# danieleschmidt/DiffFE-Physics-Lab

Measured on NVIDIA B200. Metric: fem_fwd_adjoint_solves_per_s, higher is better.
Workload: dtype f64

## Files before the change

difffe_physics_lab_b200/csrc/dfe_1d_pipe.cu:

```cuda
#include <cstdint>
#include <cstdlib>

#include "dfe_internal.h"

namespace {

#include "dfe_1d_common.cuh"

constexpr unsigned long long SENT = 0xFFFFFFFFFFFFFFFFull;
constexpr int NLMAX = 4;
constexpr int MISC_BYTES = 4096;

struct PP {
  int nn, G, chg, NG, slotd;
  long long B;
  const double* hs;
  const double* rh;
  const double* X;
  const double* in0;
  long long ld0;
  const double* in1;
  long long ld1;
  double* out;
  long long ldo;
// ... 64 lines not shown
        const long long t0 = clock64();
        while (clock64() - t0 < backoff) {}
      }
    }
  }
  s = __longlong_as_double(static_cast<long long>(a));
  m = __longlong_as_double(static_cast<long long>(b));
}

constexpr long long WAIT_LIMIT = 4000000000ll;
__device__ __forceinline__ bool mbar_try(uint64_t* bar, uint32_t parity) {
  uint32_t ok;
  asm volatile(
      "{\n\t.reg .pred p;\n\t"
      "mbarrier.try_wait.parity.shared::cta.b64 p, [%1], %2;\n\t"
      "selp.u32 %0, 1, 0, p;\n\t}"
      : "=r"(ok)
      : "r"(smem_u32(bar)), "r"(parity)
      : "memory");
  return ok != 0;
}
__device__ __forceinline__ bool mbar_test(uint64_t* bar, uint32_t parity) {
  uint32_t ok;
  asm volatile(
      "{\n\t.reg .pred p;\n\t"
      "mbarrier.test_wait.parity.shared::cta.b64 p, [%1], %2;\n\t"
      "selp.u32 %0, 1, 0, p;\n\t}"
      : "=r"(ok)
      : "r"(smem_u32(bar)), "r"(parity)
      : "memory");
  return ok != 0;
}
__device__ __noinline__ void mbar_wait_slow(uint64_t* bar, uint32_t parity, int* err, int* dead) {
  const long long t0 = clock64();
  int spins = 0;
  while (!mbar_try(bar, parity)) {
    if ((++spins & 63) == 0) {
      if (*reinterpret_cast<volatile int*>(dead)) return;
      if (clock64() - t0 > WAIT_LIMIT) {
        *reinterpret_cast<volatile int*>(dead) = 1;
        *reinterpret_cast<volatile int*>(err) = 1;
        return;
      }
    }
  }
}
__device__ __forceinline__ void mbar_wait_b(uint64_t* bar, uint32_t parity, int* err, int* dead) {
  if (!mbar_test(bar, parity)) mbar_wait_slow(bar, parity, err, dead);
}
__device__ __forceinline__ void mbar_arrive(uint64_t* bar) {
  asm volatile("mbarrier.arrive.shared::cta.b64 _, [%0];" ::"r"(smem_u32(bar)) : "memory");
}

template <bool BWD, int R, bool FULL, bool MF>
__device__ __forceinline__ void phase_a(double* buf, const double* ub, const double (&hs)[R + 1], int nin, int nst,
                                        bool ownsL, double sc, double& S, double& Wc, double& Lq) {
#pragma unroll
  for (int j = 0; j < R; ++j) {
    double in;
    if (MF) {
      const double diff = (FULL || j < nst) ? ub[j] - buf[j] : 0.0;
      Lq = fma(diff, diff, Lq);
      in = (FULL || j < nin) ? sc * diff : 0.0;
      if (!FULL && j == 0 && ownsL) in = 0.0;
      if (FULL || j < nst) buf[j] = in;
    } else {
      in = (FULL || j < nin) ? buf[j] : 0.0;
    }
    double F = BWD ? in : fma(in, hs[j + 1], in * hs[j]);
    if (!FULL && j == 0 && ownsL) F = 0.0;
    if (!BWD && (FULL || j < nst)) buf[j] = Wc;
    S += F;
    Wc = fma(hs[j + 1], S, Wc);
  }
}

template <bool BWD, int R, bool FULL, bool SK, bool KEEP>
__device__ __forceinline__ void phase_b(double* buf, const double* ub, const double (&hs)[R + 1], const double (&rh)[R + 1],
                                        double X0, int nin, int nst, bool ownsL, double c0, double kaph, double a0,
                                        double b0, double& S1, double& W1, double& D) {
  double S = 0.0, Wc = 0.0;
  double kp = SK ? 0.0 : kdiv(kaph, hs[0], rh[0]);
  double t = fma(b0, X0, a0);
#pragma unroll
  for (int j = 0; j < R; ++j) {
    double g = 0.0, Wt;
    if (BWD) {
      g = (FULL || j < nin) ? buf[j] : 0.0;
      if (!FULL && j == 0 && ownsL) g = 0.0;
      Wt = Wc;
      S += g;
      Wc = fma(hs[j + 1], S, Wc);
    } else {
      Wt = (FULL || j < nst) ? buf[j] : 0.0;
    }
    const double x0 = fma(-c0, Wt, t);
    t = fma(b0, hs[j + 1], t);
    double v1;
    if (SK) {
      v1 = __dmul_rn(rh[j + 1], x0);
    } else {
      const double ki = kdiv(kaph, hs[j + 1], rh[j + 1]);
      v1 = __dmul_rn(two_sum_err(kp, ki), x0);
      kp = ki;
    }
    if (BWD) {
      const double uj = (FULL || j < nst) ? ub[j] : 0.0;
      D = fma(g + v1, uj, D);
    }
    if (KEEP && (FULL || j < nst)) buf[j] = fma(-c0, W1, x0);
    S1 += v1;
    W1 = fma(hs[j + 1], S1, W1);
  }
}

template <bool BWD, int R, bool FULL>
__device__ __forceinline__ void phase_c(double* buf, const double (&hs)[R + 1], double X0, int nst, double a1, double b1) {
  double t = fma(b1, X0, a1);
#pragma unroll
  for (int j = 0; j < R; ++j) {
    if (FULL || j < nst) {
      const double xv = buf[j] + t;
      buf[j] = BWD ? fma(xv, hs[j], xv * hs[j + 1]) : xv;
    }
    t = fma(b1, hs[j + 1], t);
  }
}

template <int W, int NR>
struct Ctl {
  uint64_t full[NR];
  uint64_t outr[NR];
  uint64_t ufull[4];
  uint64_t ufree[4];
  uint64_t tot[2][2];
  uint64_t cf[2][2];
  double cfa[2][2][2];
  double red[2][W];
  double redL[2][W];
  double sc[2][4];
  int dead;
};

template <bool BWD, int W, int NR, int LB, int LC, bool MF>
__device__ __forceinline__ void fold_warp(const PP& p, Ctl<W, NR>* ctl, double2* pt, int lane, int c, int grp, int nIt,
                                          int nTot, const int ST) {
  constexpr int WP = W | 1;
  const int LAG = ST == 0 ? LB : LB + LC;
  const int G = p.G, GP = G + 2;
  const bool LR = p.bcL && p.bcR;
  const double rXtot = 1.0 / p.Xtot;
  const bool lift = (!BWD && ST == 0);
  const double ga = (lift && LR) ? (p.gR - p.gL) * rXtot : 0.0;
  const double gb = lift ? (p.bcL ? p.gL : p.gR) : 0.0;
  const long long sstep = p.NG;
  long long sF = grp + static_cast<long long>(1 - LAG) * sstep;
  long long sP = grp + static_cast<long long>(ST == 0 ? 0 : -LB) * sstep;
  const bool ends = BWD && c == 0;
  double ccur = 0.0, khcur = 0.0, uLcur = 0.0, uRcur = 0.0;
  {
    const int f = 1 - LAG;
    if (f >= 0 && f < nIt) {
      const double* ck = p.ck + (p.per_sample ? 2 * sF : 0);
      ccur = ck[0];
      khcur = ck[1];
      if (ends) { uLcur = p.in1[sF * p.ld1]; uRcur = p.in1[sF * p.ld1 + p.nn - 1]; }
    }
  }
  if (lane == 0) mbar_arrive(&ctl->cf[ST][0]);

  for (int it = 0; it < nTot; ++it) {
    const int par = it & 1, nxt = par ^ 1;
    const uint32_t ph = (it >> 1) & 1;
    const int f = it + 1 - LAG;
    const bool vf = f >= 0 && f < nIt;
    const unsigned long long* base = p.part + ((sF * 2 + ST) * G) * 2;
    unsigned long long ra[3], rb[3];
#pragma unroll
    for (int l = 0; l < 3; ++l) {
      const int ci = lane + 32 * l;
      ra[l] = rb[l] = SENT;
      if (vf && ci < G) ld_pair(base + 2 * ci, ra[l], rb[l]);
    }
    double cnx = 0.0, khnx = 0.0, uLnx = 0.0, uRnx = 0.0;
    if (f + 1 >= 0 && f + 1 < nIt) {
      const long long sN = sF + sstep;
      const double* ck = p.ck + (p.per_sample ? 2 * sN : 0);
      cnx = ck[0];
      khnx = ck[1];
      if (ends) { uLnx = p.in1[sN * p.ld1]; uRnx = p.in1[sN * p.ld1 + p.nn - 1]; }
    }
    mbar_wait_b(&ctl->tot[ST][par], ph, p.err, &ctl->dead);
    {
      double2* P = pt + static_cast<size_t>(ST * 2 + par) * (32 * WP) + lane * WP;
      double es[W], em[W];
      double rs = 0.0, rm = 0.0;
#pragma unroll
      for (int k = 0; k < W; ++k) {
// ... 28 lines not shown
        for (int d = 16; d > 0; d >>= 1) a += __shfl_xor_sync(0xffffffffu, a, d);
        if (jp >= 0 && jp < nIt && lane == 0) p.gkpart[sP * GP + c] = a;
      }
    }
    if (vf) {
      double Sx = 0.0, Mx = 0.0, St = 0.0, Mt = 0.0;
#pragma unroll
      for (int l = 0; l < 3; ++l) {
        const int ci = lane + 32 * l;
        if (ci < G) {
          double sv, mv;
          poll_pair(base + 2 * ci, ra[l], rb[l], sv, mv, p.err, &ctl->dead, p.backoff);
          St += sv; Mt += mv;
          if (ci < c) { Sx += sv; Mx += mv; }
        }
      }
      for (int l0 = 96; l0 < G; l0 += 32) {
        const int ci = lane + l0;
        if (ci < G) {
          double sv, mv;
          poll_pair(base + 2 * ci, SENT, SENT, sv, mv, p.err, &ctl->dead, p.backoff);
          St += sv; Mt += mv;
          if (ci < c) { Sx += sv; Mx += mv; }
        }
      }
#pragma unroll
      for (int d = 16; d > 0; d >>= 1) {
        Sx += __shfl_xor_sync(0xffffffffu, Sx, d);
        Mx += __shfl_xor_sync(0xffffffffu, Mx, d);
        St += __shfl_xor_sync(0xffffffffu, St, d);
        Mt += __shfl_xor_sync(0xffffffffu, Mt, d);
      }
      const double cc = ccur;
      const double Wtot = fma(St, p.Xtot, Mt);
      const double C = LR ? Wtot * rXtot : (p.bcL ? St : 0.0);
      const double A = gb + (p.bcL ? 0.0 : cc * Wtot) - cc * Mx;
      const double Bc = ga + cc * (C - Sx);
      if (lane == 0) {
        ctl->cfa[ST][nxt][0] = A;
        ctl->cfa[ST][nxt][1] = Bc;
        ctl->sc[nxt][2 * ST] = cc;
        if (ST == 0) ctl->sc[nxt][1] = khcur;
        if (ends) p.gkpart[sF * GP + G + ST] = C * (uRcur - uLcur) - St * uRcur;
      }
    }
    ccur = cnx; khcur = khnx; uLcur = uLnx; uRcur = uRnx;
    sF += sstep;
    sP += sstep;
    __syncwarp();
    if (lane == 0) mbar_arrive(&ctl->cf[ST][nxt]);
  }
}

template <bool BWD, int R, int W, int LB, int LC, bool SK, bool MF, bool OUT, int PF>
__global__ void __launch_bounds__(32 * (W + 3), (W >= 8 ? 1 : 2)) k1d_pipe(const PP p) {
  constexpr int LCO = OUT ? LC : 0;
  constexpr int NR = LB + LCO + 2 + PF;
  constexpr int NRU = MF ? LB + 2 : 2;
  static_assert(W <= 16 && LB >= 1 && LC >= 1 && NRU <= 4 && (!MF || BWD) && (OUT || BWD), "layout");
  static_assert(sizeof(Ctl<W, NR>) <= MISC_BYTES, "misc region");
  extern __shared__ __align__(16) unsigned char smem_raw[];
  Ctl<W, NR>* ctl = reinterpret_cast<Ctl<W, NR>*>(smem_raw);
  constexpr int WP = W | 1;
  double* ring = reinterpret_cast<double*>(smem_raw + MISC_BYTES);
  double* uring = ring + static_cast<size_t>(NR) * p.slotd;
  double2* pt = reinterpret_cast<double2*>(uring + static_cast<size_t>(BWD ? NRU : 0) * p.slotd);

  const int tid = threadIdx.x, lane = tid & 31, warp = tid >> 5;
  const int G = p.G, nn = p.nn;
  const int c = blockIdx.x % G, grp = blockIdx.x / G;
  const int n0 = c * p.chg;
  const int len = min(nn, n0 + p.chg) - n0;
  const int nIt = static_cast<int>((p.B - grp + p.NG - 1) / p.NG);
  const int nTot = nIt + LB + LC;
  const bool have_out = OUT && (p.out != nullptr);
  const int slotd = p.slotd;
  const int mis0c = static_cast<int>(((reinterpret_cast<uintptr_t>(p.in0) >> 3) + n0) & 1);
  const int mis1c = BWD ? static_cast<int>(((reinterpret_cast<uintptr_t>(p.in1) >> 3) + n0) & 1) : 0;
  const int ld0p = static_cast<int>(p.ld0 & 1), ld1p = static_cast<int>(p.ld1 & 1), ngp = p.NG & 1, grpp = grp & 1;
  auto mis0_of = [&](int j) { return mis0c ^ (ld0p & (grpp ^ (j & ngp))); };
  auto mis1_of = [&](int j) { return mis1c ^ (ld1p & (grpp ^ (j & ngp))); };

  if (tid == 0) {
    for (int k = 0; k < NR; ++k) { mbar_init_raw(&ctl->full[k], 1); mbar_init_raw(&ctl->outr[k], W); }
    for (int k = 0; k < 4; ++k) {
      mbar_init_raw(&ctl->ufull[k], 1);
      mbar_init_raw(&ctl->ufree[k], W);
    }
    for (int k = 0; k < 2; ++k)
      for (int s = 0; s < 2; ++s) { mbar_init_raw(&ctl->tot[s][k], W); mbar_init_raw(&ctl->cf[s][k], 1); }
    fence_mbar_init();
    ctl->dead = 0;
  }
  __syncthreads();

  if (warp < W) {
    const int tb = tid * R;
    const int nin = max(0, min(R, min(len, nn - (p.bcR ? 1 : 0) - n0) - tb));
    const int nst = max(0, min(R, len - tb));
    const bool ownsL = p.bcL && c == 0 && tid == 0;
    const bool ownsR = p.bcR && c == G - 1 && tb <= len - 1 && len - 1 < tb + R;
    const bool full = __all_sync(0xffffffffu, (nin == R) && (nst == R) && !ownsL && !ownsR);
    double hs[R + 1], rh[R + 1];
#pragma unroll
    for (int j = 0; j <= R; ++j) {
      const int e = n0 - 1 + tb + j;
      const bool ex = (e >= 0 && e < nn - 1 && tb + j <= len);
      hs[j] = ex ? p.hs[e] : 0.0;
      rh[j] = ex ? p.rh[e] : 0.0;
    }
    if (SK) {
      const double kaph = 0.5 * p.kappa[0];
      double kp = kdiv(kaph, hs[0], rh[0]);
#pragma unroll
      for (int j = 0; j < R; ++j) {
        const double ki = kdiv(kaph, hs[j + 1], rh[j + 1]);
        rh[j + 1] = two_sum_err(kp, ki);
        kp = ki;
      }
    }
    const double X0 = p.X[min(n0 + tb, nn - 1)];
    const double Xe = p.X[min(n0 + min(tb + R, len), nn - 1)];
    double q0s[LB - 1], q0m[LB - 1], q1s[LC - 1], q1m[LC - 1];
#pragma unroll
    for (int k = 0; k < LB - 1; ++k) q0s[k] = q0m[k] = 0.0;
#pragma unroll
    for (int k = 0; k < LC - 1; ++k) q1s[k] = q1m[k] = 0.0;
    const int pidx = (tid / W) * WP + tid % W;
    double2* pt0 = pt + pidx;
    double2* pt1 = pt + 2 * 32 * WP + pidx;

    int slotA = 0, roundA = 0;
    for (int it = 0; it < nTot; ++it) {
      const int par = it & 1;
      const uint32_t ph = (it >> 1) & 1;
      {
        double S = 0.0, Wc = 0.0, Lq = 0.0;
        if (it < nIt) {
          double* buf = ring + slotA * slotd + mis0_of(it) + tb;
          mbar_wait_b(&ctl->full[slotA], roundA, p.err, &ctl->dead);
          const double* ub = nullptr;
          if (MF) {
            const int us = it % NRU;
            ub = uring + us * slotd + mis1_of(it) + tb;
            mbar_wait_b(&ctl->ufull[us], (it / NRU) & 1, p.err, &ctl->dead);
          }
          if (full) phase_a<BWD, R, true, MF>(buf, ub, hs, nin, nst, ownsL, p.mf_scale, S, Wc, Lq);
          else phase_a<BWD, R, false, MF>(buf, ub, hs, nin, nst, ownsL, p.mf_scale, S, Wc, Lq);
        }
        pt0[par * 32 * WP] = make_double2(S, fma(-S, Xe, Wc));
        if (MF) {
#pragma unroll
          for (int d = 16; d > 0; d >>= 1) Lq += __shfl_xor_sync(0xffffffffu, Lq, d);
          if (lane == 0) ctl->redL[par][warp] = Lq;
        }
        __syncwarp();
        if (lane == 0) mbar_arrive(&ctl->tot[0][par]);
      }
      {
        const int jB = it - LB;
        int slotB = slotA - LB;
        if (slotB < 0) slotB += NR;
        double S1 = 0.0, W1 = 0.0, D = 0.0;
        mbar_wait_b(&ctl->cf[0][par], ph, p.err, &ctl->dead);
        const bool act = jB >= 0 && jB < nIt;
        if (act) {
          double* buf = ring + slotB * slotd + mis0_of(jB) + tb;
          const double c0 = ctl->sc[par][0], kaph = ctl->sc[par][1];
          const double a0 = fma(-c0, q0m[LB - 2], ctl->cfa[0][par][0]);
          const double b0 = fma(-c0, q0s[LB - 2], ctl->cfa[0][par][1]);
          const double* ub = nullptr;
          if (BWD) {
            const int us = jB % NRU;
            ub = uring + us * slotd + mis1_of(jB) + tb;
            mbar_wait_b(&ctl->ufull[us], (jB / NRU) & 1, p.err, &ctl->dead);
          }
          if (full) phase_b<BWD, R, true, SK, OUT>(buf, ub, hs, rh, X0, nin, nst, ownsL, c0, kaph, a0, b0, S1, W1, D);
          else phase_b<BWD, R, false, SK, OUT>(buf, ub, hs, rh, X0, nin, nst, ownsL, c0, kaph, a0, b0, S1, W1, D);
          if (!OUT && MF) fence_async_smem();
        }
        {
          const double2 e0 = pt0[(par ^ 1) * 32 * WP];
#pragma unroll
          for (int k = LB - 2; k > 0; --k) { q0s[k] = q0s[k - 1]; q0m[k] = q0m[k - 1]; }
          q0s[0] = e0.x;
          q0m[0] = e0.y;
        }
        pt1[par * 32 * WP] = make_double2(S1, fma(-S1, Xe, W1));
        if (BWD) {
#pragma unroll
          for (int d = 16; d > 0; d >>= 1) D += __shfl_xor_sync(0xffffffffu, D, d);
          if (lane == 0) ctl->red[par][warp] = D;
        }
        __syncwarp();
        if (lane == 0) {
          mbar_arrive(&ctl->tot[1][par]);
          if (BWD && act) mbar_arrive(&ctl->ufree[jB % NRU]);
          if (!OUT && act) mbar_arrive(&ctl->outr[slotB]);
        }
      }
      {
        const int jC = it - LB - LC;
        mbar_wait_b(&ctl->cf[1][par], ph, p.err, &ctl->dead);
        if (OUT && jC >= 0 && jC < nIt) {
          int slotC = slotA - LB - LC;
          if (slotC < 0) slotC += NR;
          if (have_out) {
            double* buf = ring + slotC * slotd + mis0_of(jC) + tb;
            const double c1 = ctl->sc[par][2];
            const double a1 = fma(-c1, q1m[LC - 2], ctl->cfa[1][par][0]);
            const double b1 = fma(-c1, q1s[LC - 2], ctl->cfa[1][par][1]);
            if (full) {
              phase_c<BWD, R, true>(buf, hs, X0, nst, a1, b1);
            } else {
              phase_c<BWD, R, false>(buf, hs, X0, nst, a1, b1);
              if (ownsL) buf[0] = BWD ? 0.0 : p.gL;
              if (ownsR) buf[len - 1 - tb] = BWD ? 0.0 : p.gR;
            }
            fence_async_smem();
          }
          __syncwarp();
          if (lane == 0) mbar_arrive(&ctl->outr[slotC]);
        }
        {
          const double2 e1 = pt1[(par ^ 1) * 32 * WP];
#pragma unroll
          for (int k = LC - 2; k > 0; --k) { q1s[k] = q1s[k - 1]; q1m[k] = q1m[k - 1]; }
          q1s[0] = e1.x;
          q1m[0] = e1.y;
        }
      }
      if (++slotA == NR) { slotA = 0; roundA ^= 1; }
    }
  } else if (warp <= W + 1) {
    fold_warp<BWD, W, NR, LB, LC, MF>(p, ctl, pt, lane, c, grp, nIt, nTot, warp - W);
  } else {
    const long long last_s = p.B - 1;
    auto load_row = [&](const double* rowbase, long long ld, long long s, double* dst, uint64_t* mb) {
      const double* g = rowbase + s * ld + n0;
      const int mis = static_cast<int>((reinterpret_cast<uintptr_t>(g) >> 3) & 1);
      int cnt = (mis + len + 1) & ~1;
      const bool clip = (s == last_s && c == G - 1 && ((mis + len) & 1));
      if (clip) cnt -= 2;
      if (lane == 0) {
        if (clip) dst[mis + len - 1] = g[len - 1];
        mbar_arrive_expect_tx(mb, 8u * static_cast<uint32_t>(cnt));
        if (cnt) bulk_g2s(dst, g - mis, 8u * cnt, mb);
      }
    };
    for (int j = 0; j < NR && j < nIt; ++j)
      load_row(p.in0, p.ld0, grp + static_cast<long long>(j) * p.NG, ring + j * slotd, &ctl->full[j]);
    if (BWD)
      for (int j = 0; j < NRU && j < nIt; ++j)
        load_row(p.in1, p.ld1, grp + static_cast<long long>(j) * p.NG, uring + j * slotd, &ctl->ufull[j]);

    int slotC = 0, roundC = 0;
    for (int it = LB; it < nTot; ++it) {
      if (BWD) {
        const int jb = it - LB;
        if (jb < nIt) {
          const int us = jb % NRU;
          mbar_wait_b(&ctl->ufree[us], (jb / NRU) & 1, p.err, &ctl->dead);
          if (jb + NRU < nIt)
            load_row(p.in1, p.ld1, grp + static_cast<long long>(jb + NRU) * p.NG, uring + us * slotd, &ctl->ufull[us]);
        }
      }
      const int jc = it - LB - LCO;
      if (jc >= 0 && jc < nIt) {
        mbar_wait_b(&ctl->outr[slotC], roundC, p.err, &ctl->dead);
        if (have_out) {
          const long long s = grp + static_cast<long long>(jc) * p.NG;
          double* go = p.out + s * p.ldo + n0;
          const double* ssrc = ring + slotC * slotd;
          const Seg qo = make_seg(go, len);
          if (lane == 0) {
            if (qo.body) bulk_s2g(go + qo.head, ssrc + qo.mis + qo.head, 8u * qo.body);
            bulk_commit();
          } else if (lane == 1) {
            if (qo.head) go[0] = ssrc[qo.mis];
          } else if (lane == 2) {
            if (qo.tail) go[len - 1] = ssrc[qo.mis + len - 1];
          }
          if (lane == 0) bulk_wait_read0();
          __syncwarp();
        }
        if (jc + NR < nIt)
          load_row(p.in0, p.ld0, grp + static_cast<long long>(jc + NR) * p.NG, ring + slotC * slotd, &ctl->full[slotC]);
        if (++slotC == NR) { slotC = 0; roundC ^= 1; }
      }
    }
    if (lane == 0) bulk_wait_all0();
  }
}

__global__ void k1d_pipe_ck(const double* kappa, long long n, double* ck, unsigned* ticket) {
  const long long s = blockIdx.x * static_cast<long long>(blockDim.x) + threadIdx.x;
  if (s == 0) *ticket = 0u;
  if (s < n) {
    const double k = kappa[s];
    ck[2 * s] = 2.0 / k;
    ck[2 * s + 1] = 0.5 * k;
  }
}

constexpr int GK_SPB = 1024;
__global__ void __launch_bounds__(256) k1d_pipe_gk(const double* part, const double* lpart, const double* kappa,
                                                   long long B, int GP, int G, int per_sample, double lsc, double* out,
                                                   double* loss_out, double* blk, unsigned* ticket) {
  if (per_sample) {
    const long long s = blockIdx.x * static_cast<long long>(blockDim.x) + threadIdx.x;
    if (s < B) {
      double a = 0.0;
      for (int g = 0; g < GP; ++g) a += part[s * GP + g];
      out[s] = -a / kappa[s];
      if (lpart) {
        double q = 0.0;
        for (int c = 0; c < G; ++c) q += lpart[s * G + c];
        loss_out[s] = lsc * q;
      }
    }
    return;
  }
  __shared__ double sh[2][256];
  __shared__ int is_last;
  const int tid = threadIdx.x;
  double a = 0.0, l = 0.0;
  for (int k = 0; k < GK_SPB / 256; ++k) {
    const long long s = static_cast<long long>(blockIdx.x) * GK_SPB + k * 256 + tid;
    if (s < B) {
      double r = 0.0;
      for (int g = 0; g < GP; ++g) r += part[s * GP + g];
      a += r;
      if (lpart) {
        double q = 0.0;
        for (int c = 0; c < G; ++c) q += lpart[s * G + c];
        l += q;
      }
    }
  }
  sh[0][tid] = a;
  sh[1][tid] = l;
  __syncthreads();
  for (int d = 128; d > 0; d >>= 1) {
    if (tid < d) { sh[0][tid] += sh[0][tid + d]; sh[1][tid] += sh[1][tid + d]; }
// ... 1 lines not shown
  }
  if (tid == 0) {
    blk[2 * blockIdx.x] = sh[0][0];
    blk[2 * blockIdx.x + 1] = sh[1][0];
    __threadfence();
    is_last = (atomicAdd(ticket, 1u) == gridDim.x - 1) ? 1 : 0;
  }
  __syncthreads();
  if (is_last && tid < 32) {
    __threadfence();
    double A = 0.0, Lt = 0.0;
    for (unsigned b = tid; b < gridDim.x; b += 32) {
      A += __ldcg(blk + 2 * b);
      Lt += __ldcg(blk + 2 * b + 1);
    }
#pragma unroll
    for (int d = 16; d > 0; d >>= 1) {
      A += __shfl_xor_sync(0xffffffffu, A, d);
      Lt += __shfl_xor_sync(0xffffffffu, Lt, d);
    }
    if (tid == 0) {
      out[0] = -A / kappa[0];
      if (loss_out) loss_out[0] = lsc * Lt;
      *ticket = 0u;
    }
  }
}

__global__ void k1d_pipe_poison(const int* err, int* err_host, double* out, long long ldo, long long B, int nn,
                                double* gk, long long ngk, double* loss, long long nloss) {
  __shared__ int bad;
  if (threadIdx.x == 0) bad = *reinterpret_cast<const volatile int*>(err);
  __syncthreads();
  if (!bad) return;
  if (threadIdx.x == 0) *reinterpret_cast<volatile int*>(err_host) = 1;
  const double nan = __longlong_as_double(0x7FF8000000000000ll);
  const long long stride = static_cast<long long>(gridDim.x) * blockDim.x;
  const long long t0 = blockIdx.x * static_cast<long long>(blockDim.x) + threadIdx.x;
  if (out)
    for (long long i = t0; i < B * nn; i += stride) out[(i / nn) * ldo + i % nn] = nan;
  if (gk)
    for (long long i = t0; i < ngk; i += stride) gk[i] = nan;
  if (loss)
    for (long long i = t0; i < nloss; i += stride) loss[i] = nan;
}

struct Geo {
  int G, chg, NG, slotd;
  size_t smem;
};

template <bool BWD, int R, int W, int LB, int LC, bool SK = false, bool MF = false, bool OUT = true, int PF = 1>
int run_cfg(const dfe_mesh* m, PP p, cudaStream_t st, int gbound, int* G_used, unsigned* ticket) {
  constexpr int NR = LB + (OUT ? LC : 0) + 2 + PF, NRU = BWD ? (MF ? LB + 2 : 2) : 0;
  constexpr int CAP = R * 32 * W, THREADS = 32 * (W + 3);
  auto kern = k1d_pipe<BWD, R, W, LB, LC, SK, MF, OUT, PF>;
  const int nn = p.nn;
  DFE_CUDA_OK(cudaFuncSetAttribute(kern, cudaFuncAttributeMaxDynamicSharedMemorySize, 227 * 1024));
  Geo g{};
  bool found = false;
  for (int per_sm = 2; per_sm >= 1 && !found; --per_sm) {
    const long long slots = static_cast<long long>(per_sm) * m->sm_count;
    const long long gcap = slots < gbound ? slots : gbound;
    const long long gmin = (nn + CAP - 1) / CAP;
    if (gmin > gcap) continue;
    long long NGmax = slots / gmin;
    if (NGmax > p.B) NGmax = p.B;
    for (long long NG = NGmax; NG >= 1 && !found; --NG) {
      long long G = slots / NG;
      if (G > gcap) G = gcap;
      if (G > nn) G = nn;
      if (p.B <= NG) G = gmin;
      g.chg = static_cast<int>((nn + G - 1) / G);
      g.chg = ((g.chg + 32 * R - 1) / (32 * R)) * (32 * R);
      if (g.chg > CAP) g.chg = CAP;
      g.G = (nn + g.chg - 1) / g.chg;
      g.NG = static_cast<int>(NG);
      g.slotd = ((g.chg + 2) + 1) & ~1;
      g.smem = MISC_BYTES + sizeof(double) * static_cast<size_t>(NR + NRU) * g.slotd + 4 * 32 * (W | 1) * 16;
      if (g.smem > 227 * 1024) continue;
      int occ = 0;
      DFE_CUDA_OK(cudaOccupancyMaxActiveBlocksPerMultiprocessor(&occ, kern, THREADS, g.smem));
      found = occ >= per_sm;
    }
  }
  if (!found) {
    dfe::set_error("dfe_solve1d (pipelined): no resident configuration for a mesh of %d nodes", nn);
    return DFE_ERR_UNSUPPORTED;
  }
  p.G = g.G;
  p.chg = g.chg;
  p.NG = g.NG;
  p.slotd = g.slotd;
  *G_used = g.G;
  DFE_CUDA_OK(cudaMemsetAsync(p.part, 0xFF, static_cast<size_t>(p.B) * 2 * g.G * 2 * sizeof(double), st));
  {
    const long long nk = p.per_sample ? p.B : 1;
    k1d_pipe_ck<<<static_cast<unsigned>((nk + 255) / 256), 256, 0, st>>>(p.kappa, nk, const_cast<double*>(p.ck), ticket);
  }
  static const bool plain_launch = getenv("DFE_PIPE_PLAIN_LAUNCH") != nullptr;
  if (plain_launch) {
    kern<<<static_cast<unsigned>(g.NG * g.G), THREADS, g.smem, st>>>(p);
    DFE_CUDA_OK(cudaGetLastError());
  } else {
    cudaLaunchConfig_t cfg{};
    cfg.gridDim = dim3(static_cast<unsigned>(g.NG * g.G));
    cfg.blockDim = dim3(THREADS);
    cfg.dynamicSmemBytes = g.smem;
    cfg.stream = st;
    cudaLaunchAttribute at[1];
    at[0].id = cudaLaunchAttributeCooperative;
    at[0].val.cooperative = 1;
    cfg.attrs = at;
    cfg.numAttrs = 1;
    DFE_CUDA_OK(cudaLaunchKernelEx(&cfg, kern, p));
  }
  return DFE_OK;
}

int cfg_id() {
  static const int id = [] {
    const char* e = getenv("DFE_PIPE_CFG");
    return e ? atoi(e) : 0;
  }();
  return id;
}

}

namespace dfe {

static size_t g_bound(const dfe_mesh* m) {
  const size_t gmin = (static_cast<size_t>(m->info.n_nodes) + 1279) / 1280;
  const size_t b = 2 * gmin + 2;
  return b < 32 * NLMAX ? b : 32 * NLMAX;
}

// ... 15 lines not shown

size_t pipe1d_workspace_bytes(const dfe_mesh* m, long long B) { return ws_layout(m, B).total; }

bool pipe1d_eligible(const dfe_mesh* m, long long B, int kappa_mode, int n_refine, const double* in0, long long ld0,
                     const double* in1, const double* out, long long ldo) {
  if (!m->chain || n_refine != 1) return false;
  if (kappa_mode != DFE_KAPPA_SCALAR && kappa_mode != DFE_KAPPA_PER_SAMPLE) return false;
  if (m->info.n_nodes > 5LL * 256 * 32 * NLMAX) return false;
  if ((reinterpret_cast<uintptr_t>(in0) | reinterpret_cast<uintptr_t>(in1)) & 15) return false;
  if (out) {
    const uintptr_t a = reinterpret_cast<uintptr_t>(in0) >> 3, b = reinterpret_cast<uintptr_t>(out) >> 3;
    if ((a ^ b) & 1) return false;
    if (B > 1 && ((ld0 ^ ldo) & 1)) return false;
  }
  return true;
}

int pipe1d_run(const dfe_mesh* m, long long B, bool bwd, const double* in0, long long ld0, const double* in1,
               long long ld1, const double* kappa, int kappa_mode, double* out, long long ldo, double* gkappa,
               void* ws, cudaStream_t st, const Misfit1D* misfit) {
  PP p{};
  p.nn = static_cast<int>(m->info.n_nodes);
  p.B = B;
  p.hs = m->d_hs;
  p.rh = m->d_rh;
  p.X = m->d_X;
  p.Xtot = m->x_total;
  p.in0 = in0; p.ld0 = ld0; p.in1 = in1; p.ld1 = ld1; p.out = out; p.ldo = ldo;
  p.kappa = kappa;
  p.per_sample = kappa_mode == DFE_KAPPA_PER_SAMPLE;
  p.bcL = m->bc_left; p.bcR = m->bc_right; p.gL = m->g_left; p.gR = m->g_right;
  const size_t gmax = g_bound(m);
  unsigned char* w = static_cast<unsigned char*>(ws);
  const WsLayout L = ws_layout(m, B);
  p.part = reinterpret_cast<unsigned long long*>(w + L.part);
  p.gkpart = reinterpret_cast<double*>(w + L.gkpart);
  p.ck = reinterpret_cast<double*>(w + L.ck);
  p.losspart = reinterpret_cast<double*>(w + L.losspart);
  p.mf_scale = misfit ? misfit->scale : 0.0;
  double* blk = reinterpret_cast<double*>(w + L.blk);
  unsigned* ticket = reinterpret_cast<unsigned*>(w + L.ticket);
  p.err = m->d_fault_dev;
  int rc, G = 0;
  const int id = cfg_id();
  static const int backoff = [] { const char* e = getenv("DFE_PIPE_BACKOFF"); return e ? atoi(e) : 0; }();
  p.backoff = backoff;
  static const bool no_sk = getenv("DFE_PIPE_NOSK") != nullptr;
  const bool sk = !p.per_sample && !no_sk;
  const int gb = static_cast<int>(gmax);
  if (!bwd) {
    switch (id) {
      case 1: rc = run_cfg<false, 11, 10, 2, 2>(m, p, st, gb, &G, ticket); break;
      case 4: rc = run_cfg<false, 9, 10, 3, 2>(m, p, st, gb, &G, ticket); break;
      default:
        rc = run_cfg<false, 9, 12, 2, 2>(m, p, st, gb, &G, ticket);
        break;
    }
  } else if (misfit) {
    if (!out) {
      switch (id) {
        case 1: rc = !sk ? run_cfg<true, 9, 10, 2, 2, false, true, false>(m, p, st, gb, &G, ticket)
                         : run_cfg<true, 9, 10, 2, 2, true, true, false>(m, p, st, gb, &G, ticket); break;
        case 2: rc = !sk ? run_cfg<true, 9, 8, 2, 2, false, true>(m, p, st, gb, &G, ticket)
                         : run_cfg<true, 9, 8, 2, 2, true, true>(m, p, st, gb, &G, ticket); break;
        default: rc = !sk ? run_cfg<true, 11, 8, 2, 2, false, true, false>(m, p, st, gb, &G, ticket)
                          : run_cfg<true, 11, 8, 2, 2, true, true, false>(m, p, st, gb, &G, ticket); break;
      }
    } else {
      rc = !sk ? run_cfg<true, 9, 8, 2, 2, false, true>(m, p, st, gb, &G, ticket)
               : run_cfg<true, 9, 8, 2, 2, true, true>(m, p, st, gb, &G, ticket);
    }
  } else if (!out) {
    switch (id) {
      case 2: rc = !sk ? run_cfg<true, 11, 8, 2, 2>(m, p, st, gb, &G, ticket)
                       : run_cfg<true, 11, 8, 2, 2, true>(m, p, st, gb, &G, ticket); break;
      case 1: rc = !sk ? run_cfg<true, 11, 10, 2, 2, false, false, false>(m, p, st, gb, &G, ticket)
                       : run_cfg<true, 11, 10, 2, 2, true, false, false>(m, p, st, gb, &G, ticket); break;
      default: rc = !sk ? run_cfg<true, 11, 8, 2, 2, false, false, false>(m, p, st, gb, &G, ticket)
                        : run_cfg<true, 11, 8, 2, 2, true, false, false>(m, p, st, gb, &G, ticket); break;
    }
  } else {
    switch (id) {
      case 1: rc = run_cfg<true, 9, 11, 2, 2>(m, p, st, gb, &G, ticket); break;
      default:
        rc = !sk ? run_cfg<true, 11, 8, 2, 2>(m, p, st, gb, &G, ticket)
                 : run_cfg<true, 11, 8, 2, 2, true>(m, p, st, gb, &G, ticket);
        break;
    }
  }
  if (rc != DFE_OK) return rc;
  if (bwd) {
    const unsigned nb = p.per_sample ? static_cast<unsigned>((B + 255) / 256) : static_cast<unsigned>((B + GK_SPB - 1) / GK_SPB);
    k1d_pipe_gk<<<nb, 256, 0, st>>>(p.gkpart, misfit ? p.losspart : nullptr, kappa, B, G + 2, G, p.per_sample,
                                    0.5 * p.mf_scale, gkappa, misfit ? misfit->loss : nullptr, blk, ticket);
    DFE_CUDA_OK(cudaGetLastError());
  }
  const long long nk = p.per_sample ? B : 1;
  return poison1d_launch(m, out, ldo, B, p.nn, bwd ? gkappa : nullptr, nk, misfit ? misfit->loss : nullptr, nk, st);
}

int poison1d_launch(const dfe_mesh* m, double* out, long long ldo, long long B, int nn, double* gk, long long ngk,
                    double* loss, long long nloss, cudaStream_t st) {
  k1d_pipe_poison<<<1, 1024, 0, st>>>(m->d_fault_dev, m->d_fault, out, ldo, B, nn, gk, ngk, loss, nloss);
  DFE_CUDA_OK(cudaGetLastError());
  return DFE_OK;
}

}
```

Measured before the change: 1.237 million.

## Stage pipeline intermediates in tensor memory instead of shared-memory ring

Per-row intermediate values carried between the pipeline phases (the prefix-sum keep vector and the z vector) are now written to Blackwell tensor memory with tcgen05.st/ld, not kept in a deep shared-memory ring. This cuts the input ring to 2+PF slots, adds separate double-buffered output slots with ofull/ofree barriers, and lets the loader refill input slots as soon as phase A releases them. The kernel is forced to one CTA per SM (launch bounds and a shared-memory floor) so the tensor-memory allocation cannot fail. The cost is tcgen05 load/store and wait latency plus lower occupancy for small-W configurations. It also adds new tile configuration cases.

```diff
diff --git a/difffe_physics_lab_b200/csrc/dfe_1d_pipe.cu b/difffe_physics_lab_b200/csrc/dfe_1d_pipe.cu
--- a/difffe_physics_lab_b200/csrc/dfe_1d_pipe.cu
+++ b/difffe_physics_lab_b200/csrc/dfe_1d_pipe.cu
@@ -140,9 +140,75 @@
   asm volatile("mbarrier.arrive.shared::cta.b64 _, [%0];" ::"r"(smem_u32(bar)) : "memory");
 }
 
+__device__ __forceinline__ void tm_st2(uint32_t a, const uint32_t* r) {
+  asm volatile("tcgen05.st.sync.aligned.32x32b.x2.b32 [%0], {%1, %2};" ::"r"(a), "r"(r[0]), "r"(r[1]) : "memory");
+}
+__device__ __forceinline__ void tm_st4(uint32_t a, const uint32_t* r) {
+  asm volatile("tcgen05.st.sync.aligned.32x32b.x4.b32 [%0], {%1, %2, %3, %4};" ::"r"(a), "r"(r[0]), "r"(r[1]), "r"(r[2]),
+               "r"(r[3]) : "memory");
+}
+__device__ __forceinline__ void tm_st8(uint32_t a, const uint32_t* r) {
+  asm volatile("tcgen05.st.sync.aligned.32x32b.x8.b32 [%0], {%1, %2, %3, %4, %5, %6, %7, %8};" ::"r"(a), "r"(r[0]),
+               "r"(r[1]), "r"(r[2]), "r"(r[3]), "r"(r[4]), "r"(r[5]), "r"(r[6]), "r"(r[7]) : "memory");
+}
+__device__ __forceinline__ void tm_st16(uint32_t a, const uint32_t* r) {
+  asm volatile("tcgen05.st.sync.aligned.32x32b.x16.b32 [%0], {%1, %2, %3, %4, %5, %6, %7, %8, %9, %10, %11, %12, %13, "
+               "%14, %15, %16};" ::"r"(a), "r"(r[0]), "r"(r[1]), "r"(r[2]), "r"(r[3]), "r"(r[4]), "r"(r[5]), "r"(r[6]),
+               "r"(r[7]), "r"(r[8]), "r"(r[9]), "r"(r[10]), "r"(r[11]), "r"(r[12]), "r"(r[13]), "r"(r[14]), "r"(r[15])
+               : "memory");
+}
+__device__ __forceinline__ void tm_ld2(uint32_t a, uint32_t* r) {
+  asm volatile("tcgen05.ld.sync.aligned.32x32b.x2.b32 {%0, %1}, [%2];" : "=r"(r[0]), "=r"(r[1]) : "r"(a) : "memory");
+}
+__device__ __forceinline__ void tm_ld4(uint32_t a, uint32_t* r) {
+  asm volatile("tcgen05.ld.sync.aligned.32x32b.x4.b32 {%0, %1, %2, %3}, [%4];" : "=r"(r[0]), "=r"(r[1]), "=r"(r[2]),
+               "=r"(r[3]) : "r"(a) : "memory");
+}
+__device__ __forceinline__ void tm_ld8(uint32_t a, uint32_t* r) {
+  asm volatile("tcgen05.ld.sync.aligned.32x32b.x8.b32 {%0, %1, %2, %3, %4, %5, %6, %7}, [%8];" : "=r"(r[0]), "=r"(r[1]),
+               "=r"(r[2]), "=r"(r[3]), "=r"(r[4]), "=r"(r[5]), "=r"(r[6]), "=r"(r[7]) : "r"(a) : "memory");
+}
+__device__ __forceinline__ void tm_ld16(uint32_t a, uint32_t* r) {
+  asm volatile("tcgen05.ld.sync.aligned.32x32b.x16.b32 {%0, %1, %2, %3, %4, %5, %6, %7, %8, %9, %10, %11, %12, %13, %14, "
+               "%15}, [%16];" : "=r"(r[0]), "=r"(r[1]), "=r"(r[2]), "=r"(r[3]), "=r"(r[4]), "=r"(r[5]), "=r"(r[6]),
+               "=r"(r[7]), "=r"(r[8]), "=r"(r[9]), "=r"(r[10]), "=r"(r[11]), "=r"(r[12]), "=r"(r[13]), "=r"(r[14]),
+               "=r"(r[15]) : "r"(a) : "memory");
+}
+template <int N>
+__device__ __forceinline__ void tm_st(uint32_t a, const uint32_t* r) {
+  if constexpr (N >= 16) { tm_st16(a, r); tm_st<N - 16>(a + 16, r + 16); }
+  else if constexpr (N >= 8) { tm_st8(a, r); tm_st<N - 8>(a + 8, r + 8); }
+  else if constexpr (N >= 4) { tm_st4(a, r); tm_st<N - 4>(a + 4, r + 4); }
+  else if constexpr (N == 2) { tm_st2(a, r); }
+}
+template <int N>
+__device__ __forceinline__ void tm_ld(uint32_t a, uint32_t* r) {
+  if constexpr (N >= 16) { tm_ld16(a, r); tm_ld<N - 16>(a + 16, r + 16); }
+  else if constexpr (N >= 8) { tm_ld8(a, r); tm_ld<N - 8>(a + 8, r + 8); }
+  else if constexpr (N >= 4) { tm_ld4(a, r); tm_ld<N - 4>(a + 4, r + 4); }
+  else if constexpr (N == 2) { tm_ld2(a, r); }
+}
+template <int R>
+__device__ __forceinline__ void tm_store(uint32_t a, const double (&v)[R]) {
+  uint32_t r[2 * R];
+#pragma unroll
+  for (int j = 0; j < R; ++j) {
+    r[2 * j] = static_cast<uint32_t>(__double2loint(v[j]));
+    r[2 * j + 1] = static_cast<uint32_t>(__double2hiint(v[j]));
+  }
+  tm_st<2 * R>(a, r);
+}
+__device__ __forceinline__ double tm_val(const uint32_t* r, int j) {
+  return __hiloint2double(static_cast<int>(r[2 * j + 1]), static_cast<int>(r[2 * j]));
+}
+__device__ __forceinline__ void tm_wait_st() { asm volatile("tcgen05.wait::st.sync.aligned;" ::: "memory"); }
+__device__ __forceinline__ void tm_wait_ld() { asm volatile("tcgen05.wait::ld.sync.aligned;" ::: "memory"); }
+__device__ __forceinline__ void tm_fence_before() { asm volatile("tcgen05.fence::before_thread_sync;" ::: "memory"); }
+__device__ __forceinline__ void tm_fence_after() { asm volatile("tcgen05.fence::after_thread_sync;" ::: "memory"); }
+
 template <bool BWD, int R, bool FULL, bool MF>
-__device__ __forceinline__ void phase_a(double* buf, const double* ub, const double (&hs)[R + 1], int nin, int nst,
-                                        bool ownsL, double sc, double& S, double& Wc, double& Lq) {
+__device__ __forceinline__ void phase_a(const double* buf, const double* ub, const double (&hs)[R + 1], int nin, int nst,
+                                        bool ownsL, double sc, double& S, double& Wc, double& Lq, double (&keep)[R]) {
 #pragma unroll
   for (int j = 0; j < R; ++j) {
     double in;
@@ -151,22 +217,22 @@
       Lq = fma(diff, diff, Lq);
       in = (FULL || j < nin) ? sc * diff : 0.0;
       if (!FULL && j == 0 && ownsL) in = 0.0;
-      if (FULL || j < nst) buf[j] = in;
     } else {
       in = (FULL || j < nin) ? buf[j] : 0.0;
     }
     double F = BWD ? in : fma(in, hs[j + 1], in * hs[j]);
     if (!FULL && j == 0 && ownsL) F = 0.0;
-    if (!BWD && (FULL || j < nst)) buf[j] = Wc;
+    keep[j] = BWD ? in : Wc;
     S += F;
     Wc = fma(hs[j + 1], S, Wc);
   }
 }
 
 template <bool BWD, int R, bool FULL, bool SK, bool KEEP>
-__device__ __forceinline__ void phase_b(double* buf, const double* ub, const double (&hs)[R + 1], const double (&rh)[R + 1],
-                                        double X0, int nin, int nst, bool ownsL, double c0, double kaph, double a0,
-                                        double b0, double& S1, double& W1, double& D) {
+__device__ __forceinline__ void phase_b(const uint32_t* kr, const double* ub, const double (&hs)[R + 1],
+                                        const double (&rh)[R + 1], double X0, int nin, int nst, bool ownsL, double c0,
+                                        double kaph, double a0, double b0, double& S1, double& W1, double& D,
+                                        double (&z)[R]) {
   double S = 0.0, Wc = 0.0;
   double kp = SK ? 0.0 : kdiv(kaph, hs[0], rh[0]);
   double t = fma(b0, X0, a0);
@@ -174,13 +240,13 @@
   for (int j = 0; j < R; ++j) {
     double g = 0.0, Wt;
     if (BWD) {
-      g = (FULL || j < nin) ? buf[j] : 0.0;
+      g = (FULL || j < nin) ? tm_val(kr, j) : 0.0;
       if (!FULL && j == 0 && ownsL) g = 0.0;
       Wt = Wc;
       S += g;
       Wc = fma(hs[j + 1], S, Wc);
     } else {
-      Wt = (FULL || j < nst) ? buf[j] : 0.0;
+      Wt = (FULL || j < nst) ? tm_val(kr, j) : 0.0;
     }
     const double x0 = fma(-c0, Wt, t);
     t = fma(b0, hs[j + 1], t);
@@ -196,29 +262,32 @@
       const double uj = (FULL || j < nst) ? ub[j] : 0.0;
       D = fma(g + v1, uj, D);
     }
-    if (KEEP && (FULL || j < nst)) buf[j] = fma(-c0, W1, x0);
+    if (KEEP) z[j] = fma(-c0, W1, x0);
     S1 += v1;
     W1 = fma(hs[j + 1], S1, W1);
   }
 }
 
 template <bool BWD, int R, bool FULL>
-__device__ __forceinline__ void phase_c(double* buf, const double (&hs)[R + 1], double X0, int nst, double a1, double b1) {
+__device__ __forceinline__ void phase_c(double* buf, const uint32_t* zr, const double (&hs)[R + 1], double X0, int nst,
+                                        double a1, double b1) {
   double t = fma(b1, X0, a1);
 #pragma unroll
   for (int j = 0; j < R; ++j) {
     if (FULL || j < nst) {
-      const double xv = buf[j] + t;
+      const double xv = tm_val(zr, j) + t;
       buf[j] = BWD ? fma(xv, hs[j], xv * hs[j + 1]) : xv;
     }
     t = fma(b1, hs[j + 1], t);
   }
 }
 
-template <int W, int NR>
+template <int W, int NI, int NO>
 struct Ctl {
-  uint64_t full[NR];
-  uint64_t outr[NR];
+  uint64_t full[NI];
+  uint64_t ifree[NI];
+  uint64_t ofull[NO + (NO == 0)];
+  uint64_t ofree[NO + (NO == 0)];
   uint64_t ufull[4];
   uint64_t ufree[4];
   uint64_t tot[2][2];
@@ -227,11 +296,12 @@
   double red[2][W];
   double redL[2][W];
   double sc[2][4];
+  uint32_t tmem;
   int dead;
 };
 
-template <bool BWD, int W, int NR, int LB, int LC, bool MF>
-__device__ __forceinline__ void fold_warp(const PP& p, Ctl<W, NR>* ctl, double2* pt, int lane, int c, int grp, int nIt,
+template <bool BWD, int W, int NI, int NO, int LB, int LC, bool MF>
+__device__ __forceinline__ void fold_warp(const PP& p, Ctl<W, NI, NO>* ctl, double2* pt, int lane, int c, int grp, int nIt,
                                           int nTot, const int ST) {
   constexpr int WP = W | 1;
   const int LAG = ST == 0 ? LB : LB + LC;
@@ -366,18 +436,27 @@
   }
 }
 
+__host__ __device__ constexpr int tm_cols(int n) { return n <= 32 ? 32 : 2 * tm_cols((n + 1) / 2); }
+constexpr size_t SMEM_ONE_CTA = 116 * 1024;
+
 template <bool BWD, int R, int W, int LB, int LC, bool SK, bool MF, bool OUT, int PF>
-__global__ void __launch_bounds__(32 * (W + 3), (W >= 8 ? 1 : 2)) k1d_pipe(const PP p) {
-  constexpr int LCO = OUT ? LC : 0;
-  constexpr int NR = LB + LCO + 2 + PF;
+__global__ void __launch_bounds__(32 * (W + 3), 1) k1d_pipe(const PP p) {
+  constexpr int NI = 2 + PF;
+  constexpr int NO = OUT ? 2 : 0;
   constexpr int NRU = MF ? LB + 2 : 2;
-  static_assert(W <= 16 && LB >= 1 && LC >= 1 && NRU <= 4 && (!MF || BWD) && (OUT || BWD), "layout");
-  static_assert(sizeof(Ctl<W, NR>) <= MISC_BYTES, "misc region");
+  constexpr int NW = LB + 1, NZ = OUT ? LC + 1 : 0;
+  constexpr int CPW = (NW + NZ) * 2 * R;
+  constexpr int TCOLS = tm_cols((W + 3) / 4 * CPW);
+  static_assert(W >= 8 && W <= 16 && LB >= 1 && LC >= 1 && PF >= 0 && NRU <= 4 && (!MF || BWD) && (OUT || BWD),
+                "layout");
+  static_assert((W + 3) / 4 * CPW <= 512, "tensor memory: 512 columns per SM");
+  static_assert(sizeof(Ctl<W, NI, NO>) <= MISC_BYTES, "misc region");
   extern __shared__ __align__(16) unsigned char smem_raw[];
-  Ctl<W, NR>* ctl = reinterpret_cast<Ctl<W, NR>*>(smem_raw);
+  Ctl<W, NI, NO>* ctl = reinterpret_cast<Ctl<W, NI, NO>*>(smem_raw);
   constexpr int WP = W | 1;
-  double* ring = reinterpret_cast<double*>(smem_raw + MISC_BYTES);
-  double* uring = ring + static_cast<size_t>(NR) * p.slotd;
+  double* islot = reinterpret_cast<double*>(smem_raw + MISC_BYTES);
+  double* oslot = islot + static_cast<size_t>(NI) * p.slotd;
+  double* uring = oslot + static_cast<size_t>(NO) * p.slotd;
   double2* pt = reinterpret_cast<double2*>(uring + static_cast<size_t>(BWD ? NRU : 0) * p.slotd);
 
   const int tid = threadIdx.x, lane = tid & 31, warp = tid >> 5;
@@ -396,7 +475,8 @@
   auto mis1_of = [&](int j) { return mis1c ^ (ld1p & (grpp ^ (j & ngp))); };
 
   if (tid == 0) {
-    for (int k = 0; k < NR; ++k) { mbar_init_raw(&ctl->full[k], 1); mbar_init_raw(&ctl->outr[k], W); }
+    for (int k = 0; k < NI; ++k) { mbar_init_raw(&ctl->full[k], 1); mbar_init_raw(&ctl->ifree[k], W); }
+    for (int k = 0; k < NO; ++k) { mbar_init_raw(&ctl->ofull[k], W); mbar_init_raw(&ctl->ofree[k], 1); }
     for (int k = 0; k < 4; ++k) {
       mbar_init_raw(&ctl->ufull[k], 1);
       mbar_init_raw(&ctl->ufree[k], W);
@@ -406,7 +486,14 @@
     fence_mbar_init();
     ctl->dead = 0;
   }
+  if (warp == 0) {
+    asm volatile("tcgen05.alloc.cta_group::1.sync.aligned.shared::cta.b32 [%0], %1;" ::"r"(smem_u32(&ctl->tmem)),
+                 "n"(TCOLS) : "memory");
+    asm volatile("tcgen05.relinquish_alloc_permit.cta_group::1.sync.aligned;" ::: "memory");
+  }
+  tm_fence_before();
   __syncthreads();
+  tm_fence_after();
 
   if (warp < W) {
     const int tb = tid * R;
@@ -443,6 +530,9 @@
     const int pidx = (tid / W) * WP + tid % W;
     double2* pt0 = pt + pidx;
     double2* pt1 = pt + 2 * 32 * WP + pidx;
+    const uint32_t tbase = ctl->tmem + (static_cast<uint32_t>(32 * (warp & 3)) << 16) + static_cast<uint32_t>((warp >> 2) * CPW);
+    auto tkeep = [&](int j) { return tbase + static_cast<uint32_t>((j % NW) * 2 * R); };
+    auto tz = [&](int j) { return tbase + static_cast<uint32_t>((NW + j % (NZ > 0 ? NZ : 1)) * 2 * R); };
 
     int slotA = 0, roundA = 0;
     for (int it = 0; it < nTot; ++it) {
@@ -451,7 +541,7 @@
       {
         double S = 0.0, Wc = 0.0, Lq = 0.0;
         if (it < nIt) {
-          double* buf = ring + slotA * slotd + mis0_of(it) + tb;
+          const double* buf = islot + slotA * slotd + mis0_of(it) + tb;
           mbar_wait_b(&ctl->full[slotA], roundA, p.err, &ctl->dead);
           const double* ub = nullptr;
           if (MF) {
@@ -459,8 +549,11 @@
             ub = uring + us * slotd + mis1_of(it) + tb;
             mbar_wait_b(&ctl->ufull[us], (it / NRU) & 1, p.err, &ctl->dead);
           }
-          if (full) phase_a<BWD, R, true, MF>(buf, ub, hs, nin, nst, ownsL, p.mf_scale, S, Wc, Lq);
-          else phase_a<BWD, R, false, MF>(buf, ub, hs, nin, nst, ownsL, p.mf_scale, S, Wc, Lq);
+          double keep[R];
+          if (full) phase_a<BWD, R, true, MF>(buf, ub, hs, nin, nst, ownsL, p.mf_scale, S, Wc, Lq, keep);
+          else phase_a<BWD, R, false, MF>(buf, ub, hs, nin, nst, ownsL, p.mf_scale, S, Wc, Lq, keep);
+          __syncwarp();
+          tm_store<R>(tkeep(it), keep);
         }
         pt0[par * 32 * WP] = make_double2(S, fma(-S, Xe, Wc));
         if (MF) {
@@ -469,17 +562,21 @@
           if (lane == 0) ctl->redL[par][warp] = Lq;
         }
         __syncwarp();
-        if (lane == 0) mbar_arrive(&ctl->tot[0][par]);
+        if (lane == 0) {
+          mbar_arrive(&ctl->tot[0][par]);
+          if (it < nIt) mbar_arrive(&ctl->ifree[slotA]);
+        }
       }
       {
         const int jB = it - LB;
-        int slotB = slotA - LB;
-        if (slotB < 0) slotB += NR;
         double S1 = 0.0, W1 = 0.0, D = 0.0;
+        const bool act = jB >= 0 && jB < nIt;
         mbar_wait_b(&ctl->cf[0][par], ph, p.err, &ctl->dead);
-        const bool act = jB >= 0 && jB < nIt;
         if (act) {
-          double* buf = ring + slotB * slotd + mis0_of(jB) + tb;
+          uint32_t kr[2 * R];
+          __syncwarp();
+          tm_wait_st();
+          tm_ld<2 * R>(tkeep(jB), kr);
           const double c0 = ctl->sc[par][0], kaph = ctl->sc[par][1];
           const double a0 = fma(-c0, q0m[LB - 2], ctl->cfa[0][par][0]);
           const double b0 = fma(-c0, q0s[LB - 2], ctl->cfa[0][par][1]);
@@ -488,10 +585,13 @@
             const int us = jB % NRU;
             ub = uring + us * slotd + mis1_of(jB) + tb;
             mbar_wait_b(&ctl->ufull[us], (jB / NRU) & 1, p.err, &ctl->dead);
+            __syncwarp();
           }
-          if (full) phase_b<BWD, R, true, SK, OUT>(buf, ub, hs, rh, X0, nin, nst, ownsL, c0, kaph, a0, b0, S1, W1, D);
-          else phase_b<BWD, R, false, SK, OUT>(buf, ub, hs, rh, X0, nin, nst, ownsL, c0, kaph, a0, b0, S1, W1, D);
-          if (!OUT && MF) fence_async_smem();
+          tm_wait_ld();
+          double z[R];
+          if (full) phase_b<BWD, R, true, SK, OUT>(kr, ub, hs, rh, X0, nin, nst, ownsL, c0, kaph, a0, b0, S1, W1, D, z);
+          else phase_b<BWD, R, false, SK, OUT>(kr, ub, hs, rh, X0, nin, nst, ownsL, c0, kaph, a0, b0, S1, W1, D, z);
+          if constexpr (OUT) tm_store<R>(tz(jB), z);
         }
         {
           const double2 e0 = pt0[(par ^ 1) * 32 * WP];
@@ -510,31 +610,38 @@
         if (lane == 0) {
           mbar_arrive(&ctl->tot[1][par]);
           if (BWD && act) mbar_arrive(&ctl->ufree[jB % NRU]);
-          if (!OUT && act) mbar_arrive(&ctl->outr[slotB]);
         }
       }
       {
         const int jC = it - LB - LC;
+        const bool act = OUT && jC >= 0 && jC < nIt;
         mbar_wait_b(&ctl->cf[1][par], ph, p.err, &ctl->dead);
-        if (OUT && jC >= 0 && jC < nIt) {
-          int slotC = slotA - LB - LC;
-          if (slotC < 0) slotC += NR;
-          if (have_out) {
-            double* buf = ring + slotC * slotd + mis0_of(jC) + tb;
-            const double c1 = ctl->sc[par][2];
-            const double a1 = fma(-c1, q1m[LC - 2], ctl->cfa[1][par][0]);
-            const double b1 = fma(-c1, q1s[LC - 2], ctl->cfa[1][par][1]);
-            if (full) {
-              phase_c<BWD, R, true>(buf, hs, X0, nst, a1, b1);
-            } else {
-              phase_c<BWD, R, false>(buf, hs, X0, nst, a1, b1);
-              if (ownsL) buf[0] = BWD ? 0.0 : p.gL;
-              if (ownsR) buf[len - 1 - tb] = BWD ? 0.0 : p.gR;
+        if constexpr (OUT) {
+          if (act) {
+            const int so = jC & 1;
+            mbar_wait_b(&ctl->ofree[so], ((jC >> 1) & 1) ^ 1, p.err, &ctl->dead);
+            __syncwarp();
+            uint32_t zr[2 * R];
+            tm_wait_st();
+            tm_ld<2 * R>(tz(jC), zr);
+            tm_wait_ld();
+            if (have_out) {
+              double* buf = oslot + so * slotd + mis0_of(jC) + tb;
+              const double c1 = ctl->sc[par][2];
+              const double a1 = fma(-c1, q1m[LC - 2], ctl->cfa[1][par][0]);
+              const double b1 = fma(-c1, q1s[LC - 2], ctl->cfa[1][par][1]);
+              if (full) {
+                phase_c<BWD, R, true>(buf, zr, hs, X0, nst, a1, b1);
+              } else {
+                phase_c<BWD, R, false>(buf, zr, hs, X0, nst, a1, b1);
+                if (ownsL) buf[0] = BWD ? 0.0 : p.gL;
+                if (ownsR) buf[len - 1 - tb] = BWD ? 0.0 : p.gR;
+              }
+              fence_async_smem();
             }
-            fence_async_smem();
+            __syncwarp();
+            if (lane == 0) mbar_arrive(&ctl->ofull[so]);
           }
-          __syncwarp();
-          if (lane == 0) mbar_arrive(&ctl->outr[slotC]);
         }
         {
           const double2 e1 = pt1[(par ^ 1) * 32 * WP];
@@ -544,10 +651,10 @@
           q1m[0] = e1.y;
         }
       }
-      if (++slotA == NR) { slotA = 0; roundA ^= 1; }
+      if (++slotA == NI) { slotA = 0; roundA ^= 1; }
     }
   } else if (warp <= W + 1) {
-    fold_warp<BWD, W, NR, LB, LC, MF>(p, ctl, pt, lane, c, grp, nIt, nTot, warp - W);
+    fold_warp<BWD, W, NI, NO, LB, LC, MF>(p, ctl, pt, lane, c, grp, nIt, nTot, warp - W);
   } else {
     const long long last_s = p.B - 1;
     auto load_row = [&](const double* rowbase, long long ld, long long s, double* dst, uint64_t* mb) {
@@ -562,30 +669,37 @@
         if (cnt) bulk_g2s(dst, g - mis, 8u * cnt, mb);
       }
     };
-    for (int j = 0; j < NR && j < nIt; ++j)
-      load_row(p.in0, p.ld0, grp + static_cast<long long>(j) * p.NG, ring + j * slotd, &ctl->full[j]);
+    for (int j = 0; j < NI && j < nIt; ++j)
+      load_row(p.in0, p.ld0, grp + static_cast<long long>(j) * p.NG, islot + j * slotd, &ctl->full[j]);
     if (BWD)
       for (int j = 0; j < NRU && j < nIt; ++j)
         load_row(p.in1, p.ld1, grp + static_cast<long long>(j) * p.NG, uring + j * slotd, &ctl->ufull[j]);
 
-    int slotC = 0, roundC = 0;
-    for (int it = LB; it < nTot; ++it) {
+    int slotI = 0, roundI = 0;
+    for (int it = 0; it < nTot; ++it) {
+      if (it < nIt) {
+        mbar_wait_b(&ctl->ifree[slotI], roundI, p.err, &ctl->dead);
+        if (it + NI < nIt)
+          load_row(p.in0, p.ld0, grp + static_cast<long long>(it + NI) * p.NG, islot + slotI * slotd, &ctl->full[slotI]);
+        if (++slotI == NI) { slotI = 0; roundI ^= 1; }
+      }
       if (BWD) {
         const int jb = it - LB;
-        if (jb < nIt) {
+        if (jb >= 0 && jb < nIt) {
           const int us = jb % NRU;
           mbar_wait_b(&ctl->ufree[us], (jb / NRU) & 1, p.err, &ctl->dead);
           if (jb + NRU < nIt)
             load_row(p.in1, p.ld1, grp + static_cast<long long>(jb + NRU) * p.NG, uring + us * slotd, &ctl->ufull[us]);
         }
       }
-      const int jc = it - LB - LCO;
-      if (jc >= 0 && jc < nIt) {
-        mbar_wait_b(&ctl->outr[slotC], roundC, p.err, &ctl->dead);
+      const int jc = it - LB - LC;
+      if (OUT && jc >= 0 && jc < nIt) {
+        const int so = jc & 1;
+        mbar_wait_b(&ctl->ofull[so], (jc >> 1) & 1, p.err, &ctl->dead);
         if (have_out) {
           const long long s = grp + static_cast<long long>(jc) * p.NG;
           double* go = p.out + s * p.ldo + n0;
-          const double* ssrc = ring + slotC * slotd;
+          const double* ssrc = oslot + so * slotd;
           const Seg qo = make_seg(go, len);
           if (lane == 0) {
             if (qo.body) bulk_s2g(go + qo.head, ssrc + qo.mis + qo.head, 8u * qo.body);
@@ -598,12 +712,16 @@
           if (lane == 0) bulk_wait_read0();
           __syncwarp();
         }
-        if (jc + NR < nIt)
-          load_row(p.in0, p.ld0, grp + static_cast<long long>(jc + NR) * p.NG, ring + slotC * slotd, &ctl->full[slotC]);
-        if (++slotC == NR) { slotC = 0; roundC ^= 1; }
+        if (lane == 0) mbar_arrive(&ctl->ofree[so]);
       }
     }
     if (lane == 0) bulk_wait_all0();
+  }
+  tm_fence_before();
+  __syncthreads();
+  if (warp == 0) {
+    tm_fence_after();
+    asm volatile("tcgen05.dealloc.cta_group::1.sync.aligned.b32 %0, %1;" ::"r"(ctl->tmem), "n"(TCOLS) : "memory");
   }
 }
 
@@ -711,37 +829,35 @@
 
 template <bool BWD, int R, int W, int LB, int LC, bool SK = false, bool MF = false, bool OUT = true, int PF = 1>
 int run_cfg(const dfe_mesh* m, PP p, cudaStream_t st, int gbound, int* G_used, unsigned* ticket) {
-  constexpr int NR = LB + (OUT ? LC : 0) + 2 + PF, NRU = BWD ? (MF ? LB + 2 : 2) : 0;
+  constexpr int NSLOT = (2 + PF) + (OUT ? 2 : 0) + (BWD ? (MF ? LB + 2 : 2) : 0);
   constexpr int CAP = R * 32 * W, THREADS = 32 * (W + 3);
   auto kern = k1d_pipe<BWD, R, W, LB, LC, SK, MF, OUT, PF>;
   const int nn = p.nn;
   DFE_CUDA_OK(cudaFuncSetAttribute(kern, cudaFuncAttributeMaxDynamicSharedMemorySize, 227 * 1024));
   Geo g{};
   bool found = false;
-  for (int per_sm = 2; per_sm >= 1 && !found; --per_sm) {
-    const long long slots = static_cast<long long>(per_sm) * m->sm_count;
-    const long long gcap = slots < gbound ? slots : gbound;
-    const long long gmin = (nn + CAP - 1) / CAP;
-    if (gmin > gcap) continue;
-    long long NGmax = slots / gmin;
-    if (NGmax > p.B) NGmax = p.B;
-    for (long long NG = NGmax; NG >= 1 && !found; --NG) {
-      long long G = slots / NG;
-      if (G > gcap) G = gcap;
-      if (G > nn) G = nn;
-      if (p.B <= NG) G = gmin;
-      g.chg = static_cast<int>((nn + G - 1) / G);
-      g.chg = ((g.chg + 32 * R - 1) / (32 * R)) * (32 * R);
-      if (g.chg > CAP) g.chg = CAP;
-      g.G = (nn + g.chg - 1) / g.chg;
-      g.NG = static_cast<int>(NG);
-      g.slotd = ((g.chg + 2) + 1) & ~1;
-      g.smem = MISC_BYTES + sizeof(double) * static_cast<size_t>(NR + NRU) * g.slotd + 4 * 32 * (W | 1) * 16;
-      if (g.smem > 227 * 1024) continue;
-      int occ = 0;
-      DFE_CUDA_OK(cudaOccupancyMaxActiveBlocksPerMultiprocessor(&occ, kern, THREADS, g.smem));
-      found = occ >= per_sm;
-    }
+  const long long slots = m->sm_count;
+  const long long gcap = slots < gbound ? slots : gbound;
+  const long long gmin = (nn + CAP - 1) / CAP;
+  long long NGmax = gmin <= gcap ? slots / gmin : 0;
+  if (NGmax > p.B) NGmax = p.B;
+  for (long long NG = NGmax; NG >= 1 && !found; --NG) {
+    long long G = slots / NG;
+    if (G > gcap) G = gcap;
+    if (G > nn) G = nn;
+    if (p.B <= NG) G = gmin;
+    g.chg = static_cast<int>((nn + G - 1) / G);
+    g.chg = ((g.chg + 32 * R - 1) / (32 * R)) * (32 * R);
+    if (g.chg > CAP) g.chg = CAP;
+    g.G = (nn + g.chg - 1) / g.chg;
+    g.NG = static_cast<int>(NG);
+    g.slotd = ((g.chg + 2) + 1) & ~1;
+    g.smem = MISC_BYTES + sizeof(double) * static_cast<size_t>(NSLOT) * g.slotd + 4 * 32 * (W | 1) * 16;
+    if (g.smem > 227 * 1024) continue;
+    if (g.smem < SMEM_ONE_CTA) g.smem = SMEM_ONE_CTA;
+    int occ = 0;
+    DFE_CUDA_OK(cudaOccupancyMaxActiveBlocksPerMultiprocessor(&occ, kern, THREADS, g.smem));
+    found = occ >= 1;
   }
   if (!found) {
     dfe::set_error("dfe_solve1d (pipelined): no resident configuration for a mesh of %d nodes", nn);
@@ -863,6 +979,9 @@
     switch (id) {
       case 1: rc = run_cfg<false, 11, 10, 2, 2>(m, p, st, gb, &G, ticket); break;
       case 4: rc = run_cfg<false, 9, 10, 3, 2>(m, p, st, gb, &G, ticket); break;
+      case 5: rc = run_cfg<false, 11, 12, 2, 2>(m, p, st, gb, &G, ticket); break;
+      case 6: rc = run_cfg<false, 12, 12, 2, 2>(m, p, st, gb, &G, ticket); break;
+      case 7: rc = run_cfg<false, 9, 12, 2, 2, false, false, true, 2>(m, p, st, gb, &G, ticket); break;
       default:
         rc = run_cfg<false, 9, 12, 2, 2>(m, p, st, gb, &G, ticket);
         break;
@@ -893,6 +1012,8 @@
   } else {
     switch (id) {
       case 1: rc = run_cfg<true, 9, 11, 2, 2>(m, p, st, gb, &G, ticket); break;
+      case 5: rc = run_cfg<true, 11, 10, 2, 2>(m, p, st, gb, &G, ticket); break;
+      case 6: rc = run_cfg<true, 9, 12, 2, 2>(m, p, st, gb, &G, ticket); break;
       default:
         rc = !sk ? run_cfg<true, 11, 8, 2, 2>(m, p, st, gb, &G, ticket)
                  : run_cfg<true, 11, 8, 2, 2, true>(m, p, st, gb, &G, ticket);
```

New measurement: 1.280 million (median of 6 runs). 3.4% higher.
